# PhucNguyenAH/tacotron2_subword

Measured on AMD Instinct MI355X. Metric: mel_frames_per_sec_train, higher is better.
Workload: dtype bf16; 1 GPU; BERT_Tacotron2 default hparams (SMA), full training iteration fwd+loss+bwd+clip+Adam, B=64/GPU, 100 phones, 60 sub-word tokens, 400 frames, 80-mel; global_batch=64, frames_per_item=400, parallelism=dp1, torch_ops=loss reductions, cat/transpose copies, persistent_chains=True, recurrent_steps_bf16=True

## Files before the change

include/t2amd.h:

```cpp
#ifndef T2AMD_H
#define T2AMD_H
#include <stddef.h>
#include <stdint.h>

#ifdef __cplusplus
extern "C" {
#endif

#define T2_ATTN_SMA 0
#define T2_ATTN_LSA 1
#define T2_ATTN_DCA 4
#define T2_ATTN_GMM 3
#define T2_ATTN_FWD2 2

enum {
    T2_SITE_PRENET1 = 1, T2_SITE_PRENET2 = 2, T2_SITE_PRENET1_SUB = 3, T2_SITE_PRENET2_SUB = 4,
    T2_SITE_ATT_H = 5, T2_SITE_ATT_C = 6, T2_SITE_ATT_H_SUB = 7, T2_SITE_ATT_C_SUB = 8,
    T2_SITE_DEC_H = 9, T2_SITE_DEC_C = 10, T2_SITE_NOISE = 11, T2_SITE_NOISE_SUB = 12,
    T2_SITE_ENC0 = 16,
    T2_SITE_ENCSUB0 = 20,
    T2_SITE_POSTNET0 = 24
};

const char* t2_last_error(void);
#define T2_ABI_VERSION 4
int t2_version(void);
int t2_chain_status(uint32_t* out_host );
int t2_chain_status_clear(void);
int t2_debug_report_abort(uint32_t code, void* stream);
int t2_debug_occupy(int workgroups, int milliseconds, void* stream);
int t2_chain_claimed(void);
int t2_set_precision(int mode);
int t2_get_precision(void);
int t2_gemm_counts(uint64_t* out_host , int reset);
int t2_set_gemm_split_min_mflop(int mflop);
int t2_set_split_steps(int on);
int t2_get_split_steps(void);
int t2_step_counts(uint64_t* out_host , int reset);
int t2_set_overlap(int on);
int t2_set_chain(int on);
int t2_get_chain(void);
int t2_set_chain_bwd(int on);
int t2_set_gemm_staging(int on);
int t2_set_gemm_fold(int on);
int t2_set_bn_fuse(int on);
int t2_get_bn_fuse(void);
int t2_bn_fuse_counts(uint64_t* out_host , int reset);
int t2_side_join(void* stream);
int t2_defer_counts(uint64_t* out_host , int reset);

typedef struct t2_dims {
    int n_mel;
    int prenet_dim;
    int enc_dim;
    int att_rnn_dim;
    int dec_rnn_dim;
    int att_dim;
    int loc_filters;
    int loc_kernel;
    int attention_kind;
    float p_att_dropout, p_dec_dropout, p_prenet_dropout;
    int n_streams;
    float score_mask_value, score_mask_value_sub;
    int score_mask_given;
} t2_dims;

typedef struct t2_attention_weights {
// ... 159 lines not shown
    float* gates[4];
    float* ws; size_t ws_floats;
} t2_lstm_seq_args;
size_t t2_lstm_seq_chain_ws_floats(int nstreams, int B, int H, int backward);
int t2_lstm_seq_forward(const t2_lstm_seq_args* a, void* stream);
typedef struct t2_lstm_seq_bwd_args {
    int nstreams, B, T, H;
    const float* w_hh[4]; int reverse[4];
    const float* h[4]; long ldh; const float* c[4]; const float* gates[4];
    const float* dh[4]; long lddh;
    float* dpre[4];
    float* dw_hh[4];
    float* ws; size_t ws_floats;
} t2_lstm_seq_bwd_args;
int t2_lstm_seq_backward(const t2_lstm_seq_bwd_args* a, void* stream);

typedef struct t2_gemm_args {
    const float* A; const float* B; float* C; int M, N, K;
    long sam, sak, sbn, sbk, ldc; int batch; long bsA, bsB, bsC;
    float alpha, beta; const float* bias; int act; int crow_mod; long crow_mul;
    float* ws; size_t ws_bytes; int splitk;
} t2_gemm_args;
int t2_gemm_ex(const t2_gemm_args* a, void* stream);
int t2_prof_gemm(const t2_gemm_args* a, int reps, float* ms_total, float* ms_kernel, void* stream);
enum { T2_GEMM_F32_64 = 0, T2_GEMM_F32_128, T2_GEMM_BF16CONV, T2_GEMM_SRC128, T2_GEMM_SRC256, T2_GEMM_SRC256KM };
enum { T2_GEMM_OPERAND_FP32 = 0, T2_GEMM_OPERAND_STAGED, T2_GEMM_OPERAND_CALLER };
typedef struct t2_gemm_plan_opts {
    int conv_a, conv_b, conv_T, conv_C, fp32_only;
    int a16, b16; long lda16, ldb16; int a16_kmajor, b16_kmajor, split16;
} t2_gemm_plan_opts;
typedef struct t2_gemm_plan_info {
    int kernel; const char* name;
    int split;
    int splitk, kchunks;
    int a_src, b_src;
    size_t stage_bytes_a, stage_bytes_b;
} t2_gemm_plan_info;
int t2_gemm_plan(const t2_gemm_args* a, const t2_gemm_plan_opts* opts, t2_gemm_plan_info* out);
int t2_conv_handoff_plan(const t2_gemm_args* a, const t2_gemm_plan_opts* opts, int* taken, t2_gemm_plan_info* out);
int t2_colsum(const float* x, long ld, int M, int N, float* out, float* scratch, void* stream);
int t2_mask_btc(float* x, int B, int T, int C, const int32_t* lengths, float fill, void* stream);

typedef struct t2_softdtw_plan_info {
    int threads;
    int rows_per_thread;
    int passes;
// ... 133 lines not shown
```

tacotron2_subword_amd/_lib.py:

```python
from __future__ import annotations

import ctypes as C
import os

import torch

_HERE = os.path.dirname(os.path.abspath(__file__))
LIB_PATH = os.environ.get("T2AMD_LIB") or os.path.join(_HERE, "libt2amd.so")

ATTN_SMA, ATTN_LSA, ATTN_FWD2, ATTN_GMM, ATTN_DCA = 0, 1, 2, 3, 4

SITE = dict(PRENET1=1, PRENET2=2, PRENET1_SUB=3, PRENET2_SUB=4, ATT_H=5, ATT_C=6, ATT_H_SUB=7, ATT_C_SUB=8,
            DEC_H=9, DEC_C=10, NOISE=11, NOISE_SUB=12, ENC0=16, ENCSUB0=20, POSTNET0=24)

_fp = C.POINTER(C.c_float)
_ip = C.POINTER(C.c_int32)


class Dims(C.Structure):
    _fields_ = [("n_mel", C.c_int), ("prenet_dim", C.c_int), ("enc_dim", C.c_int), ("att_rnn_dim", C.c_int),
                ("dec_rnn_dim", C.c_int), ("att_dim", C.c_int), ("loc_filters", C.c_int), ("loc_kernel", C.c_int),
                ("attention_kind", C.c_int), ("p_att_dropout", C.c_float), ("p_dec_dropout", C.c_float),
                ("p_prenet_dropout", C.c_float), ("n_streams", C.c_int),
                ("score_mask_value", C.c_float), ("score_mask_value_sub", C.c_float), ("score_mask_given", C.c_int)]
# ... 99 lines not shown
_I4 = C.c_int * 4


class LstmSeqArgs(C.Structure):
    _fields_ = [("nstreams", C.c_int), ("B", C.c_int), ("T", C.c_int), ("H", C.c_int),
                ("pre", _P4), ("w_hh", _P4), ("reverse", _I4), ("lengths", C.c_void_p),
                ("h", _P4), ("ldh", C.c_long), ("c", _P4), ("gates", _P4), ("ws", C.c_void_p), ("ws_floats", C.c_size_t)]


class LstmSeqBwdArgs(C.Structure):
    _fields_ = [("nstreams", C.c_int), ("B", C.c_int), ("T", C.c_int), ("H", C.c_int),
                ("w_hh", _P4), ("reverse", _I4), ("h", _P4), ("ldh", C.c_long), ("c", _P4), ("gates", _P4),
                ("dh", _P4), ("lddh", C.c_long), ("dpre", _P4), ("dw_hh", _P4), ("ws", C.c_void_p), ("ws_floats", C.c_size_t)]


class GemmArgs(C.Structure):
    _fields_ = [("A", C.c_void_p), ("B", C.c_void_p), ("C", C.c_void_p), ("M", C.c_int), ("N", C.c_int), ("K", C.c_int),
                ("sam", C.c_long), ("sak", C.c_long), ("sbn", C.c_long), ("sbk", C.c_long), ("ldc", C.c_long),
                ("batch", C.c_int), ("bsA", C.c_long), ("bsB", C.c_long), ("bsC", C.c_long),
                ("alpha", C.c_float), ("beta", C.c_float), ("bias", C.c_void_p), ("act", C.c_int),
                ("crow_mod", C.c_int), ("crow_mul", C.c_long), ("ws", C.c_void_p), ("ws_bytes", C.c_size_t), ("splitk", C.c_int)]


class GemmPlanOpts(C.Structure):
    _fields_ = [("conv_a", C.c_int), ("conv_b", C.c_int), ("conv_T", C.c_int), ("conv_C", C.c_int), ("fp32_only", C.c_int),
                ("a16", C.c_int), ("b16", C.c_int), ("lda16", C.c_long), ("ldb16", C.c_long),
                ("a16_kmajor", C.c_int), ("b16_kmajor", C.c_int), ("split16", C.c_int)]


class GemmPlanInfo(C.Structure):
    _fields_ = [("kernel", C.c_int), ("name", C.c_char_p), ("split", C.c_int), ("splitk", C.c_int), ("kchunks", C.c_int),
                ("a_src", C.c_int), ("b_src", C.c_int), ("stage_bytes_a", C.c_size_t), ("stage_bytes_b", C.c_size_t)]


class SoftDtwPlanInfo(C.Structure):
    _fields_ = [("threads", C.c_int), ("rows_per_thread", C.c_int), ("passes", C.c_int),
                ("d_floats", C.c_size_t), ("r_floats", C.c_size_t), ("e_floats", C.c_size_t)]


class SoftDtwDistArgs(C.Structure):
    _fields_ = [("B", C.c_int), ("N", C.c_int), ("M", C.c_int), ("d", C.c_int), ("x", C.c_void_p), ("y", C.c_void_p), ("Ds", C.c_void_p)]


class SoftDtwFwdArgs(C.Structure):
    _fields_ = [("B", C.c_int), ("N", C.c_int), ("M", C.c_int), ("gamma", C.c_float), ("bandwidth", C.c_float),
                ("D", C.c_void_p), ("Ds", C.c_void_p), ("x_lengths", C.c_void_p), ("y_lengths", C.c_void_p),
# ... 43 lines not shown


class StftPlanInfo(C.Structure):
    _fields_ = [("bins", C.c_int), ("overlap", C.c_int), ("frame_tile", C.c_int), ("bin_tile", C.c_int), ("out_len", C.c_long),
                ("fwd_floats", C.c_size_t), ("inv_floats", C.c_size_t), ("wsq_floats", C.c_size_t), ("packed_bytes", C.c_size_t)]


class StftAnalysisArgs(C.Structure):
    _fields_ = [("B", C.c_int), ("N", C.c_int), ("hop", C.c_int), ("n", C.c_long), ("x", C.c_void_p), ("packed", C.c_void_p),
                ("re", C.c_void_p), ("im", C.c_void_p), ("mag", C.c_void_p), ("phase", C.c_void_p)]


class StftSynthesisArgs(C.Structure):
    _fields_ = [("B", C.c_int), ("N", C.c_int), ("hop", C.c_int), ("nf", C.c_int), ("mode", C.c_int), ("windowed", C.c_int),
                ("a", C.c_void_p), ("b", C.c_void_p), ("bias", C.c_void_p), ("strength", C.c_float),
                ("packed", C.c_void_p), ("y", C.c_void_p)]


STFT_FRAME_TILE = 32
STFT_POLAR, STFT_DENOISE = 0, 1

ABI_VERSION = 4

EXPORTS = ["t2_last_error", "t2_version", "t2_chain_status", "t2_chain_status_clear", "t2_debug_report_abort", "t2_debug_occupy", "t2_chain_claimed", "t2_set_precision", "t2_get_precision", "t2_gemm_counts", "t2_set_gemm_split_min_mflop", "t2_set_split_steps", "t2_get_split_steps", "t2_step_counts", "t2_set_overlap", "t2_set_chain", "t2_get_chain", "t2_set_chain_bwd", "t2_set_gemm_staging", "t2_set_gemm_fold", "t2_set_bn_fuse", "t2_get_bn_fuse", "t2_bn_fuse_counts", "t2_side_join", "t2_defer_counts", "t2_decoder_layout_query", "t2_decoder_forward", "t2_decoder_infer",
           "t2_decoder_bwd_layout_query", "t2_decoder_backward", "t2_prof_enable", "t2_prof_collect", "t2_adam_chunks", "t2_adam_step", "t2_adam_norm",
           "t2_conv_bn_forward", "t2_conv_bn_backward", "t2_embedding_forward", "t2_embedding_backward",
           "t2_lstm_seq_forward", "t2_lstm_seq_backward", "t2_lstm_seq_chain_ws_floats", "t2_gemm_ex", "t2_prof_gemm", "t2_gemm_plan", "t2_conv_handoff_plan", "t2_colsum", "t2_mask_btc",
           "t2_finalize_bct", "t2_mask_bt", "t2_gemm", "t2_rng_keep_mask", "t2_rng_normal",
           "t2_softdtw_plan", "t2_softdtw_dist", "t2_softdtw_forward", "t2_softdtw_backward", "t2_softdtw_dist_backward",
           "t2_hifigan_plan", "t2_hifigan_pack", "t2_hifigan_forward", "t2_vocoder_packed_floats", "t2_vocoder_conv1d", "t2_vocoder_conv_transpose1d",
           "t2_stft_plan", "t2_stft_pack", "t2_stft_analysis", "t2_stft_synthesis"]

_lib = None


def lib() -> C.CDLL:
    global _lib
    if _lib is None:
        if not os.path.exists(LIB_PATH):
            raise RuntimeError(f"{LIB_PATH} is missing: the HIP extension must be built (see __graft_entry__.build); "
                               "there is no CPU fallback for the product path")
        L = C.CDLL(LIB_PATH)
        L.t2_last_error.restype = C.c_char_p
        if L.t2_version() != ABI_VERSION:
            raise RuntimeError(f"{LIB_PATH} speaks ABI version {L.t2_version()}, this binding {ABI_VERSION}: rebuild the library "
                               "(the argument structs differ in size between versions)")
        L.t2_chain_status.argtypes = [C.POINTER(C.c_uint32)]
        L.t2_debug_report_abort.argtypes = [C.c_uint32, C.c_void_p]
        L.t2_debug_occupy.argtypes = [C.c_int, C.c_int, C.c_void_p]
        L.t2_gemm.argtypes = [C.c_void_p, C.c_void_p, C.c_void_p, C.c_int, C.c_int, C.c_int, C.c_long, C.c_long, C.c_long,
                              C.c_long, C.c_long, C.c_void_p, C.c_int, C.c_float, C.c_float, C.c_void_p, C.c_size_t,
                              C.c_int, C.c_void_p]
        L.t2_rng_keep_mask.argtypes = [C.c_uint64, C.c_uint32, C.c_uint32, C.c_float, C.c_void_p, C.c_void_p]
        L.t2_rng_normal.argtypes = [C.c_uint64, C.c_uint32, C.c_uint32, C.c_void_p, C.c_void_p]
        L.t2_decoder_layout_query.argtypes = [C.POINTER(Dims), C.c_int, C.c_int, C.c_int, C.c_int, C.POINTER(DecoderLayout)]
        L.t2_decoder_forward.argtypes = [C.POINTER(Dims), C.POINTER(DecoderWeights), C.POINTER(DecoderFwdArgs), C.c_void_p]
        L.t2_decoder_infer.argtypes = [C.POINTER(Dims), C.POINTER(DecoderWeights), C.POINTER(DecoderInferArgs), C.c_void_p]
        L.t2_decoder_bwd_layout_query.argtypes = [C.POINTER(Dims), C.c_int, C.c_int, C.c_int, C.c_int, C.POINTER(DecoderBwdLayout)]
        L.t2_decoder_backward.argtypes = [C.POINTER(Dims), C.POINTER(DecoderWeights), C.POINTER(DecoderGrads),
                                          C.POINTER(DecoderBwdArgs), C.c_void_p]
        L.t2_conv_bn_forward.argtypes = [C.POINTER(ConvBnArgs), C.c_void_p]
        L.t2_conv_bn_backward.argtypes = [C.POINTER(ConvBnBwdArgs), C.c_void_p]
        L.t2_embedding_forward.argtypes = [C.c_void_p, C.c_void_p, C.c_void_p, C.c_int, C.c_int, C.c_void_p]
        L.t2_embedding_backward.argtypes = [C.c_void_p, C.c_void_p, C.c_void_p, C.c_int, C.c_int, C.c_int, C.c_void_p]
        L.t2_lstm_seq_forward.argtypes = [C.POINTER(LstmSeqArgs), C.c_void_p]
        L.t2_lstm_seq_backward.argtypes = [C.POINTER(LstmSeqBwdArgs), C.c_void_p]
        L.t2_lstm_seq_chain_ws_floats.argtypes, L.t2_lstm_seq_chain_ws_floats.restype = [C.c_int, C.c_int, C.c_int, C.c_int], C.c_size_t
        L.t2_gemm_ex.argtypes = [C.POINTER(GemmArgs), C.c_void_p]
        L.t2_prof_gemm.argtypes = [C.POINTER(GemmArgs), C.c_int, C.POINTER(C.c_float), C.POINTER(C.c_float), C.c_void_p]
        L.t2_gemm_plan.argtypes = [C.POINTER(GemmArgs), C.POINTER(GemmPlanOpts), C.POINTER(GemmPlanInfo)]
        L.t2_conv_handoff_plan.argtypes = [C.POINTER(GemmArgs), C.POINTER(GemmPlanOpts), C.POINTER(C.c_int), C.POINTER(GemmPlanInfo)]
        L.t2_colsum.argtypes = [C.c_void_p, C.c_long, C.c_int, C.c_int, C.c_void_p, C.c_void_p, C.c_void_p]
        L.t2_mask_btc.argtypes = [C.c_void_p, C.c_int, C.c_int, C.c_int, C.c_void_p, C.c_float, C.c_void_p]
        L.t2_prof_enable.argtypes = [C.c_int]
        L.t2_gemm_counts.argtypes = [C.POINTER(C.c_uint64), C.c_int]
        L.t2_set_split_steps.argtypes = [C.c_int]
        L.t2_step_counts.argtypes = [C.POINTER(C.c_uint64), C.c_int]
        L.t2_bn_fuse_counts.argtypes = [C.POINTER(C.c_uint64), C.c_int]
        L.t2_defer_counts.argtypes = [C.POINTER(C.c_uint64), C.c_int]
        L.t2_set_gemm_split_min_mflop.argtypes = [C.c_int]
        L.t2_prof_collect.argtypes = [C.c_int, C.POINTER(C.c_double), C.POINTER(C.c_int)]
        L.t2_finalize_bct.argtypes = [C.c_void_p, C.c_void_p, C.c_int, C.c_int, C.c_int, C.c_void_p, C.c_float, C.c_void_p]
        L.t2_mask_bt.argtypes = [C.c_void_p, C.c_int, C.c_int, C.c_void_p, C.c_float, C.c_void_p]
        L.t2_softdtw_plan.argtypes = [C.c_int, C.c_int, C.c_int, C.c_float, C.c_int, C.POINTER(SoftDtwPlanInfo)]
        L.t2_softdtw_dist.argtypes = [C.POINTER(SoftDtwDistArgs), C.c_void_p]
        L.t2_softdtw_forward.argtypes = [C.POINTER(SoftDtwFwdArgs), C.c_void_p]
        L.t2_softdtw_backward.argtypes = [C.POINTER(SoftDtwBwdArgs), C.c_void_p]
        L.t2_softdtw_dist_backward.argtypes = [C.POINTER(SoftDtwDistBwdArgs), C.c_void_p]
        L.t2_hifigan_plan.argtypes = [C.POINTER(HifiganConfig), C.c_int, C.c_int, C.POINTER(HifiganPlanInfo)]
        L.t2_hifigan_pack.argtypes = [C.POINTER(HifiganConfig), C.POINTER(C.c_void_p), C.POINTER(C.c_void_p), C.c_int, C.c_void_p, C.c_void_p]
        L.t2_hifigan_forward.argtypes = [C.POINTER(HifiganConfig), C.POINTER(HifiganFwdArgs), C.c_void_p]
# ... 224 lines not shown
    out = (C.c_uint64 * 6)()
    check(lib().t2_step_counts(out, int(bool(reset))))
    return tuple(int(v) for v in out)


def gemm_plan(args: GemmArgs, **opts) -> dict:
    o, info = GemmPlanOpts(**opts), GemmPlanInfo()
    check(lib().t2_gemm_plan(C.byref(args), C.byref(o), C.byref(info)))
    return dict(kernel=info.kernel, name=info.name.decode(), split=bool(info.split), splitk=info.splitk, kchunks=info.kchunks,
                a_src=info.a_src, b_src=info.b_src, stage_bytes_a=info.stage_bytes_a, stage_bytes_b=info.stage_bytes_b)


def conv_handoff_plan(args: GemmArgs, **opts) -> dict:
    o, info, taken = GemmPlanOpts(**opts), GemmPlanInfo(), C.c_int(0)
    check(lib().t2_conv_handoff_plan(C.byref(args), C.byref(o), C.byref(taken), C.byref(info)))
    return dict(taken=bool(taken.value), kernel=info.kernel, name=info.name.decode(), split=bool(info.split), splitk=info.splitk,
                kchunks=info.kchunks, a_src=info.a_src, b_src=info.b_src, stage_bytes_a=info.stage_bytes_a, stage_bytes_b=info.stage_bytes_b)


def set_gemm_fold(on: bool) -> None:
    check(lib().t2_set_gemm_fold(1 if on else 0))


def set_bn_fuse(on: bool) -> None:
    check(lib().t2_set_bn_fuse(1 if on else 0))


def get_bn_fuse() -> bool:
    return bool(lib().t2_get_bn_fuse())


def bn_fuse_counts(reset: bool = False):
    out = (C.c_uint64 * 3)()
    check(lib().t2_bn_fuse_counts(out, int(bool(reset))))
    return tuple(int(v) for v in out)


def defer_counts(reset: bool = False):
    out = (C.c_uint64 * 2)()
    check(lib().t2_defer_counts(out, int(bool(reset))))
    return tuple(int(v) for v in out)


def set_gemm_split_min_mflop(mflop: int = -1) -> None:
    check(lib().t2_set_gemm_split_min_mflop(int(mflop)))

# ... 44 lines not shown
```

tacotron2_subword_amd/csrc/c_api.hip:

```cpp
#include <fcntl.h>
#include <stdarg.h>
#include <stdio.h>
#include <sys/file.h>
#include <unistd.h>
#include <stdlib.h>
#include <string.h>

#include "../../include/t2amd.h"
#include "kernels.h"
#include "driver.h"

static thread_local char g_err[512] = "";

void t2_set_error(const char* fmt, ...) {
    va_list ap;
    va_start(ap, fmt);
    vsnprintf(g_err, sizeof(g_err), fmt, ap);
    va_end(ap);
}

#include <algorithm>
#include <mutex>
#include <vector>

// ... 165 lines not shown
    set_precision(mode);
    return 0;
}
int t2_get_precision(void) { return get_precision(); }
int t2_set_gemm_split_min_mflop(int mflop) { set_gemm_split_min_mflop(mflop); return 0; }
int t2_gemm_counts(uint64_t* out_host, int reset) {
    T2_REQUIRE(out_host, "null argument");
    gemm_counts(out_host, reset);
    return 0;
}
int t2_set_split_steps(int on) { g_split_steps = on != 0; return 0; }
int t2_get_split_steps(void) { return g_split_steps; }
int t2_step_counts(uint64_t* out_host, int reset) {
    T2_REQUIRE(out_host, "null argument");
    for (int i = 0; i < 6; ++i) { out_host[i] = g_step_counts[i]; if (reset) g_step_counts[i] = 0; }
    return 0;
}
int t2_set_overlap(int on) { g_overlap = on != 0; return 0; }
int t2_set_chain(int on) { g_chain = on != 0; return 0; }
int t2_get_chain(void) { return g_chain; }
int t2_set_chain_bwd(int on) { g_chain_bwd = on != 0; return 0; }
int t2_set_gemm_staging(int on) { set_gemm_staging(on); return 0; }
int t2_set_gemm_fold(int on) { set_gemm_fold(on); return 0; }
int t2_set_bn_fuse(int on) { set_bn_fuse(on); return 0; }
int t2_get_bn_fuse(void) { return get_bn_fuse(); }
int t2_bn_fuse_counts(uint64_t* out_host, int reset) {
    T2_REQUIRE(out_host, "null argument");
    bn_fuse_counts(out_host, reset);
    return 0;
}
int t2_defer_counts(uint64_t* out_host, int reset) {
    T2_REQUIRE(out_host, "null argument");
    for (int i = 0; i < 2; ++i) { out_host[i] = g_defer_counts[i]; if (reset) g_defer_counts[i] = 0; }
    return 0;
}
int t2_side_join(void* stream) {
    Side* side = nullptr;
    T2_TRY(side_get(&side));
    hipEvent_t e;
    T2_TRY(side_event(*side, 0, &e));
    T2_CHECK_HIP(hipEventRecord(e, side->s));
    T2_CHECK_HIP(hipStreamWaitEvent((hipStream_t)stream, e, 0));
    return 0;
}

int t2_conv_bn_forward(const t2_conv_bn_args* a, void* stream) {
// ... 124 lines not shown
        w.A = a->reverse[i] ? a->dpre[i] : a->dpre[i] + rowsB * 4 * H; w.sam = 1; w.sak = 4 * H;
        w.B = a->reverse[i] ? a->h[i] + rowsB * a->ldh : a->h[i]; w.sbk = a->ldh; w.sbn = 1;
        w.C = a->dw_hh[i]; w.ldc = H; w.M = 4 * H; w.N = H; w.K = (T - 1) * B;
        w.ws = gws; w.ws_bytes = gws_bytes;
        T2_TRY(gemm(w, s));
    }
    return 0;
}

static GemmDesc desc_of(const t2_gemm_args& a) {
    GemmDesc g = gemm_desc();
    g.A = a.A; g.B = a.B; g.C = a.C; g.M = a.M; g.N = a.N; g.K = a.K;
    g.sam = a.sam; g.sak = a.sak; g.sbn = a.sbn; g.sbk = a.sbk; g.ldc = a.ldc;
    g.batch = a.batch > 0 ? a.batch : 1; g.bsA = a.bsA; g.bsB = a.bsB; g.bsC = a.bsC;
    g.alpha = a.alpha; g.beta = a.beta; g.bias1 = a.bias; g.act = a.act;
    g.crow_mod = a.crow_mod; g.crow_mul = a.crow_mul;
    g.ws = a.ws; g.ws_bytes = a.ws_bytes; g.splitk = a.splitk;
    return g;
}
int t2_gemm_ex(const t2_gemm_args* a, void* stream) {
    T2_REQUIRE(a, "null argument");
    return gemm(desc_of(*a), (hipStream_t)stream);
}
static GemmDesc desc_of(const t2_gemm_args& a, const t2_gemm_plan_opts* o) {
    GemmDesc g = desc_of(a);
    if (o) {
        g.conv_a = o->conv_a; g.conv_b = o->conv_b; g.conv_T = o->conv_T; g.conv_C = o->conv_C; g.fp32_only = o->fp32_only;
        const __bf16* copy = reinterpret_cast<const __bf16*>(uintptr_t(256));
        if (o->a16) { g.A16 = copy; g.lda16 = o->lda16; g.a16_kmajor = o->a16_kmajor; }
        if (o->b16) { g.B16 = copy; g.ldb16 = o->ldb16; g.b16_kmajor = o->b16_kmajor; }
        g.split16 = o->split16;
    }
    return g;
}
static t2_gemm_plan_info info_of(const GemmPlan& p) {
    return t2_gemm_plan_info{(int)p.kernel, gemm_plan_name(p), p.split, p.splitk, p.kchunks, (int)p.a.src, (int)p.b.src, p.a.bytes, p.b.bytes};
}
int t2_gemm_plan(const t2_gemm_args* a, const t2_gemm_plan_opts* o, t2_gemm_plan_info* out) {
    T2_REQUIRE(a && out, "null argument");
    GemmPlan p;
    T2_TRY(gemm_plan(desc_of(*a, o), &p));
    *out = info_of(p);
    return 0;
}
int t2_conv_handoff_plan(const t2_gemm_args* a, const t2_gemm_plan_opts* o, int* taken, t2_gemm_plan_info* out) {
    T2_REQUIRE(a && taken && out, "null argument");
// ... 208 lines not shown
```

tacotron2_subword_amd/csrc/gemm.hip:

```cpp
#include "kernels.h"
#include <cstdlib>
#include <algorithm>
#include <type_traits>

namespace t2 {

static int g_precision = 0;
static int env_int(const char* name, int dflt) { const char* v = getenv(name); return v && *v ? atoi(v) : dflt; }
static int g_stage = env_int("T2_GEMM_STAGE", 1);
void set_gemm_staging(int on) { g_stage = on != 0; }
static int g_fold = env_int("T2_GEMM_FOLD", 1);
void set_gemm_fold(int on) { g_fold = on != 0; }
int get_gemm_fold() { return g_fold; }
constexpr int kStageMin = 256;
constexpr int kSplitMinMflopDefault = 2147;
static double g_split_min_flop = 1e6 * kSplitMinMflopDefault;
void set_gemm_split_min_mflop(int mflop) { g_split_min_flop = 1e6 * (mflop < 0 ? kSplitMinMflopDefault : mflop); }
void set_precision(int p) { g_precision = p; }
int get_precision() { return g_precision; }
static uint64_t g_counts[4] = {0, 0, 0, 0};
void gemm_counts(uint64_t* out, int reset) {
    for (int i = 0; i < 4; ++i) { out[i] = g_counts[i]; if (reset) g_counts[i] = 0; }
}

namespace {

constexpr int BK = 16;

struct GemmK {
    GemmDesc d;
    int kchunks;
    int avec, bvec;
    int xcd_swizzle;
};

__device__ __forceinline__ float apply_act(float v, int act) {
// ... 214 lines not shown
        int s = 0;
        for (; s + 8 <= d.splitk; s += 8) {
            float v[8];
#pragma unroll
            for (int j = 0; j < 8; ++j) v[j] = d.ws[(long)(s + j) * total + i];
#pragma unroll
            for (int j = 0; j < 8; ++j) acc += v[j];
        }
        if (s + 4 <= d.splitk) {
            float v[4];
#pragma unroll
            for (int j = 0; j < 4; ++j) v[j] = d.ws[(long)(s + j) * total + i];
#pragma unroll
            for (int j = 0; j < 4; ++j) acc += v[j];
            s += 4;
        }
        for (; s < d.splitk; ++s) acc += d.ws[(long)s * total + i];
        const int bz = (int)(i / ((long)d.M * d.N));
        const long rem = i - (long)bz * d.M * d.N;
        const int m = (int)(rem / d.N), n = (int)(rem % d.N);
        epilogue_store<decltype(cmap)::value>(d, d.C + (long)bz * d.bsC, m, n, acc, key);
    }
    });
}


typedef __bf16 bf16x8 __attribute__((ext_vector_type(8)));
constexpr int BK16 = 64, PK16 = BK16;
__device__ __forceinline__ int swz16(int row, int slot) { return row * PK16 + ((slot ^ ((row ^ (row >> 2)) & 7)) << 3); }

__device__ __forceinline__ bf16x8 pack8(const f32x4& lo, const f32x4& hi) {
    bf16x8 v;
#pragma unroll
    for (int j = 0; j < 4; ++j) { v[j] = (__bf16)lo[j]; v[4 + j] = (__bf16)hi[j]; }
    return v;
}

__device__ __forceinline__ void load16_kc(const float* __restrict__ base, long srow, int row0, int nrows, int k0, int kend, int vec,
                                          ConvAddr cv, bf16x8 (&regs)[4]) {
    if (cv.T && row0 + 128 <= nrows && k0 + BK16 <= kend) {
        f32x4 lo[4], hi[4];
        bool ok[4];
#pragma unroll
        for (int i = 0; i < 4; ++i) {
            const int q = threadIdx.x + i * 256, row = row0 + (q >> 3), k = k0 + (q & 7) * 8;
            const int dk = k / cv.C, ci = k - dk * cv.C, t = row % cv.T + dk - cv.pad;
// ... 893 lines not shown

int choose_splitk(const GemmDesc& d, bool tile256, long tiles, int kch, size_t ws_bytes) {
    if (!(d.ws && d.beta == 0.f)) return 1;
    int sp = 1;
    if (tile256) {
        const int nkt = kch / 4;
        if (d.splitk > 0) sp = std::min(d.splitk, std::max(1, nkt / 2));
        else if (tiles < 512) {
            double best = 0.0;
            for (int c = 1; c <= 16; ++c) {
                if (c > 1 && nkt / c < 16) break;
                const long wgs = tiles * c, rounds = (wgs + 255) / 256;
                const double eff = (double)wgs / (256.0 * rounds);
                if (eff > best * 1.05) { best = eff; sp = c; }
            }
        }
    } else if (d.splitk > 0) sp = d.splitk;
    else if (tiles < 512 && kch >= 64) sp = std::min((int)((1024 + tiles - 1) / tiles), kch / 16);
    const size_t per = (size_t)d.batch * d.M * d.N * sizeof(float);
    if ((size_t)sp * per > ws_bytes) sp = (int)(ws_bytes / per);
    return std::max(sp, 1);
}

int run_gemm(const GemmDesc& d, const GemmPlan& p, hipStream_t s) {
    GemmK g{};
    g.d = d;
    g.kchunks = p.kchunks; g.avec = p.avec; g.bvec = p.bvec;
    if (d.conv_a) { g.d.sam = 0; g.d.sak = 1; }
    if (d.conv_b) { g.d.sbk = 0; g.d.sbn = 1; }
    if (d.drop_mstride == 0) g.d.drop_mstride = (uint32_t)d.N;
    g.d.K = p.K; g.d.conv_C = p.conv_C; g.d.splitk = p.splitk;
    const size_t staged = p.a.bytes + p.b.bytes;
    if (staged) { g.d.ws = reinterpret_cast<float*>(reinterpret_cast<unsigned char*>(d.ws) + staged); g.d.ws_bytes = d.ws_bytes - staged; }
    const int tile = p.kernel == GemmKernel::f32_64 ? 64 : p.kernel >= GemmKernel::src256 ? 256 : 128;
    const dim3 grid((d.N + tile - 1) / tile, (d.M + tile - 1) / tile, d.batch * p.splitk);
    if (gemm_reads_bf16_copies(p.kernel)) {
        __bf16* a16 = reinterpret_cast<__bf16*>(d.ws), * b16 = reinterpret_cast<__bf16*>(reinterpret_cast<unsigned char*>(d.ws) + p.a.bytes);
        if (p.a.src == GemmSrc::staged) T2_TRY_RC(stage_planned(d.A, p.a, p.split, a16, s));
        if (p.b.src == GemmSrc::staged) T2_TRY_RC(stage_planned(d.B, p.b, p.split, b16, s));
        const __bf16* pa = p.a.src == GemmSrc::caller ? d.A16 : a16, * pb = p.b.src == GemmSrc::caller ? d.B16 : b16;
        if (p.kernel == GemmKernel::src256km && d.conv_b) T2_TRY_RC((launch_bf16src256<false, true, true>(g, pa, p.a.ld, pb, p.b.ld, grid, s)));
        else if (p.kernel == GemmKernel::src256km) T2_TRY_RC((launch_bf16src256<false, true, false>(g, pa, p.a.ld, pb, p.b.ld, grid, s)));
        else if (p.kernel == GemmKernel::src256 && d.conv_a) T2_TRY_RC((launch_bf16src256<true, false, false>(g, pa, p.a.ld, pb, p.b.ld, grid, s)));
        else if (p.kernel == GemmKernel::src256) T2_TRY_RC((launch_bf16src256<false, false, false>(g, pa, p.a.ld, pb, p.b.ld, grid, s)));
        else if (d.conv_a) T2_TRY_RC((launch_bf16src<true, 2, 2, 2, 2, 2>(g, pa, p.a.ld, pb, p.b.ld, grid, s)));
        else T2_TRY_RC((launch_bf16src<false, 2, 2, 2, 2, 2>(g, pa, p.a.ld, pb, p.b.ld, grid, s)));
    } else {
        using Kernel = void (*)(GemmK);
        static const Kernel bf16conv[] = {gemm_bf16_kernel<true, true>, gemm_bf16_kernel<true, false>, gemm_bf16_kernel<false, true>, gemm_bf16_kernel<false, false>};
        static const Kernel f32_64[] = {gemm_kernel<64, 64, true, true>, gemm_kernel<64, 64, true, false>, gemm_kernel<64, 64, false, true>, gemm_kernel<64, 64, false, false>};
        static const Kernel f32_128[] = {gemm_kernel<128, 128, true, true>, gemm_kernel<128, 128, true, false>, gemm_kernel<128, 128, false, true>, gemm_kernel<128, 128, false, false>};
        const bool conv16 = p.kernel == GemmKernel::bf16conv;
        const size_t smem = conv16 ? (size_t)4 * 128 * PK16 * sizeof(__bf16) : 0;
        const Kernel kernel = (conv16 ? bf16conv : p.kernel == GemmKernel::f32_64 ? f32_64 : f32_128)[(g.d.sak == 1 ? 0 : 2) + (g.d.sbk == 1 ? 0 : 1)];
        hipLaunchKernelGGL(kernel, grid, dim3(256), smem, s, g);
    }
    T2_LAUNCH_CHECK();
    if (p.splitk > 1) {
        const long total = (long)d.batch * d.M * d.N;
        int blocks = (int)((total + 255) / 256);
        if (blocks > 2048) blocks = 2048;
        hipLaunchKernelGGL(splitk_reduce_kernel, dim3(blocks), dim3(256), 0, s, g.d);
        T2_LAUNCH_CHECK();
    }
    return 0;
}

}

int stage_bf16(const float* src, bool kc, long ld, __bf16* dst, int rows, int K, hipStream_t s) {
    T2_REQUIRE(rows > 0 && K > 0 && rows % 64 == 0 && K % 64 == 0 && ld % 4 == 0 && aligned16(src) && aligned16(dst),
               "stage_bf16: rows=%d K=%d ld=%ld must be whole 64-tiles of 16-byte aligned rows", rows, K, ld);
    return stage_operand(src, kc, ld, dst, rows, K, s);
}

int stage_split_bf16(const float* src, bool kc, long ld, __bf16* dst, int rows, int K, int lo_slot, int row_group, hipStream_t s) {
    T2_REQUIRE(rows > 0 && K > 0 && rows % 64 == 0 && K % 64 == 0 && ld % 4 == 0 && aligned16(src) && aligned16(dst) &&
               (lo_slot == 1 || lo_slot == 2) && row_group >= 0 && (!row_group || (kc && rows % row_group == 0)),
               "stage_split_bf16: rows=%d K=%d ld=%ld must be whole 64-tiles of 16-byte aligned rows", rows, K, ld);
    return stage_split_operand(src, kc, ld, dst, rows, K, lo_slot, row_group, s);
}

int stage_planned(const float* src, const GemmOperandPlan& o, bool split, __bf16* dst, hipStream_t s) {
    return split ? stage_split_operand(src, o.kc, o.ld_src, dst, o.rows, o.K, o.lo_slot, o.row_group, s)
                 : stage_operand(src, o.kc, o.ld_src, dst, o.rows, o.K, s);
}

// ... 81 lines not shown
    T2_TRY_RC(check_gemm(d));
    *out = plan_gemm(d);
    T2_REQUIRE((long)d.batch * out->splitk <= 65535, "gemm: batch*splitk too large (%d*%d)", d.batch, out->splitk);
    return 0;
}

bool gemm_handoff(const GemmDesc& plain, const GemmDesc& offered, GemmPlan* plan) {
    const GemmPlan p0 = plan_gemm(plain);
    if (plan) *plan = p0;
    if (g_precision != 1 || !gemm_reads_bf16_copies(p0.kernel) || !(offered.A16 || offered.B16)) return false;
    if ((offered.A16 && p0.a.src != GemmSrc::staged) || (offered.B16 && p0.b.src != GemmSrc::staged)) return false;
    const GemmPlan p1 = plan_gemm(offered);
    if (p1.kernel != p0.kernel || p1.split != p0.split || p1.splitk != p0.splitk || p1.kchunks != p0.kchunks) return false;
    if ((offered.A16 && p1.a.src != GemmSrc::caller) || (offered.B16 && p1.b.src != GemmSrc::caller)) return false;
    if (plan) *plan = p1;
    return true;
}

int gemm(const GemmDesc& d, hipStream_t s) {
    GemmPlan p;
    T2_TRY_RC(gemm_plan(d, &p));
    static const int g_log = env_int("T2_GEMM_LOG", 0);
    if (g_log)
        fprintf(stderr, "t2gemm M=%d N=%d K=%d batch=%d %s%s kernel=%s splitk=%d stageA=%d stageB=%d convA=%d convB=%d beta=%g\n", d.M, d.N, d.K, d.batch,
                d.conv_a || d.sak == 1 ? "A[m][k]" : "A[k][m]", !d.conv_b && d.sbk == 1 ? " B[n][k]" : " B[k][n]", gemm_plan_name(p),
                p.splitk, p.a.src == GemmSrc::staged, p.b.src == GemmSrc::staged, d.conv_a, d.conv_b, (double)d.beta);
    ++g_counts[p.split ? 3 : gemm_reads_bf16_copies(p.kernel) ? 2 : p.kernel == GemmKernel::bf16conv ? 1 : 0];
    return run_gemm(d, p, s);
}

}
```

tacotron2_subword_amd/csrc/kernels.h:

```cpp
#pragma once
#include "common.h"

namespace t2 {

enum Act : int { ACT_NONE = 0, ACT_RELU = 1, ACT_TANH = 2 };

struct GemmDesc {
    const float* A; const float* B; float* C;
    int M, N, K;
    long sam, sak;
    long sbn, sbk;
    long ldc;
    int batch; long bsA, bsB, bsC;
    float alpha, beta;
    const float* bias1; const float* bias2;
    int act;
    float drop_p; uint64_t seed; uint32_t site;
    uint32_t drop_base, drop_mstride;
    float* ws; size_t ws_bytes;
    int splitk;
    int conv_a, conv_b, conv_T, conv_C, conv_pad;
    int fp32_only;
    const __bf16* A16; long lda16;
    const __bf16* B16; long ldb16;
// ... 25 lines not shown
};
struct GemmPlan {
    GemmKernel kernel;
    bool split;
    int splitk, kchunks;
    int K, conv_C;
    GemmOperandPlan a, b;
    int avec, bvec;
};
GemmPlan plan_gemm(const GemmDesc& d);
int gemm_plan(const GemmDesc& d, GemmPlan* out);
bool gemm_handoff(const GemmDesc& plain, const GemmDesc& offered, GemmPlan* plan = nullptr);
const char* gemm_plan_name(const GemmPlan& p);
int stage_planned(const float* src, const GemmOperandPlan& o, bool split, __bf16* dst, hipStream_t s);
int stage_bf16(const float* src, bool kc, long ld, __bf16* dst, int rows, int K, hipStream_t s);
int stage_split_bf16(const float* src, bool kc, long ld, __bf16* dst, int rows, int K, int lo_slot, int row_group, hipStream_t s);
void set_precision(int p);
int get_precision();
void gemm_counts(uint64_t* out, int reset);
void set_gemm_split_min_mflop(int mflop);
void set_gemm_staging(int on);
void set_gemm_fold(int on);
int get_gemm_fold();

constexpr int kMaxSeg = 6;
struct LstmSeg { const float* x; long ldx; const float* w; long ldw; int k; };
struct LstmStream {
    LstmSeg seg[kMaxSeg]; int nseg;
    const float* pre; long ldpre;
    const float* bias1; const float* bias2;
    const float* c_prev; long ldc_prev;
    float* gates; long ldgates;
    float* c_new; long ldc_new;
    float* h_out; long ldh_out;
    float* h_out2; long ldh_out2;
    float* c_out; long ldc_out;
    uint32_t site_h, site_c; uint32_t idx_base, idx_bstride;
    const int* lengths; int t;
    const float* wq; int A; float* qpart;
    const __bf16* x16; long ldx16; const __bf16* w16; long ldw16; int k16;
    __bf16* h16_out; long ldh16;
    __bf16* h16_out2; long ldh16_2;
    const float* xs; long ldxs; const __bf16* w16lo;
};
constexpr int kMaxLstmStreams = 4;
struct LstmStepDesc { LstmStream st[kMaxLstmStreams]; int nstreams; int B, H; float drop_p; uint64_t seed; };
// ... 345 lines not shown
```

Baseline: 1.056 million mel-frames/s.

## Add vectorized wide and column-mapped split-K reduction kernels

Replaces the scalar split-K reduction with a planner that picks a float4-vectorized kernel which sums several partial slabs per thread with unrolled loads. A second variant handles column-remapped outputs by reordering results through shared memory so stores stay coalesced. Both target the memory-bound reduction pass that follows split-K GEMMs. An env/API toggle keeps the old path available, and a standalone reduce entry point is exposed. The new kernels add more template instantiations and alignment conditions that decide which path runs.

New measurement: 1.061 million mel-frames/s, median of 6. No clear change (+0.5%).

```diff
diff --git a/include/t2amd.h b/include/t2amd.h
--- a/include/t2amd.h
+++ b/include/t2amd.h
@@ -43,6 +43,7 @@
 int t2_set_chain_bwd(int on);
 int t2_set_gemm_staging(int on);
 int t2_set_gemm_fold(int on);
+int t2_set_splitk_reduce(int wide);
 int t2_set_bn_fuse(int on);
 int t2_get_bn_fuse(void);
 int t2_bn_fuse_counts(uint64_t* out_host , int reset);
@@ -248,6 +249,13 @@
     float* ws; size_t ws_bytes; int splitk;
 } t2_gemm_args;
 int t2_gemm_ex(const t2_gemm_args* a, void* stream);
+typedef struct t2_splitk_reduce_opts {
+    const float* bias2; const float* r1_m; const float* r1_n;
+    float drop_p; uint64_t seed; uint32_t site, drop_base, drop_mstride;
+    int ccol_mod, ccol_mul;
+} t2_splitk_reduce_opts;
+int t2_splitk_reduce(const t2_gemm_args* a, int splitk, void* stream);
+int t2_splitk_reduce_ex(const t2_gemm_args* a, const t2_splitk_reduce_opts* opts, int splitk, void* stream);
 int t2_prof_gemm(const t2_gemm_args* a, int reps, float* ms_total, float* ms_kernel, void* stream);
 enum { T2_GEMM_F32_64 = 0, T2_GEMM_F32_128, T2_GEMM_BF16CONV, T2_GEMM_SRC128, T2_GEMM_SRC256, T2_GEMM_SRC256KM };
 enum { T2_GEMM_OPERAND_FP32 = 0, T2_GEMM_OPERAND_STAGED, T2_GEMM_OPERAND_CALLER };
diff --git a/tacotron2_subword_amd/_lib.py b/tacotron2_subword_amd/_lib.py
--- a/tacotron2_subword_amd/_lib.py
+++ b/tacotron2_subword_amd/_lib.py
@@ -145,6 +145,12 @@
                 ("crow_mod", C.c_int), ("crow_mul", C.c_long), ("ws", C.c_void_p), ("ws_bytes", C.c_size_t), ("splitk", C.c_int)]
 
 
+class SplitkReduceOpts(C.Structure):
+    _fields_ = [("bias2", C.c_void_p), ("r1_m", C.c_void_p), ("r1_n", C.c_void_p),
+                ("drop_p", C.c_float), ("seed", C.c_uint64), ("site", C.c_uint32), ("drop_base", C.c_uint32), ("drop_mstride", C.c_uint32),
+                ("ccol_mod", C.c_int), ("ccol_mul", C.c_int)]
+
+
 class GemmPlanOpts(C.Structure):
     _fields_ = [("conv_a", C.c_int), ("conv_b", C.c_int), ("conv_T", C.c_int), ("conv_C", C.c_int), ("fp32_only", C.c_int),
                 ("a16", C.c_int), ("b16", C.c_int), ("lda16", C.c_long), ("ldb16", C.c_long),
@@ -234,10 +240,10 @@
 
 ABI_VERSION = 4
 
-EXPORTS = ["t2_last_error", "t2_version", "t2_chain_status", "t2_chain_status_clear", "t2_debug_report_abort", "t2_debug_occupy", "t2_chain_claimed", "t2_set_precision", "t2_get_precision", "t2_gemm_counts", "t2_set_gemm_split_min_mflop", "t2_set_split_steps", "t2_get_split_steps", "t2_step_counts", "t2_set_overlap", "t2_set_chain", "t2_get_chain", "t2_set_chain_bwd", "t2_set_gemm_staging", "t2_set_gemm_fold", "t2_set_bn_fuse", "t2_get_bn_fuse", "t2_bn_fuse_counts", "t2_side_join", "t2_defer_counts", "t2_decoder_layout_query", "t2_decoder_forward", "t2_decoder_infer",
+EXPORTS = ["t2_last_error", "t2_version", "t2_chain_status", "t2_chain_status_clear", "t2_debug_report_abort", "t2_debug_occupy", "t2_chain_claimed", "t2_set_precision", "t2_get_precision", "t2_gemm_counts", "t2_set_gemm_split_min_mflop", "t2_set_split_steps", "t2_get_split_steps", "t2_step_counts", "t2_set_overlap", "t2_set_chain", "t2_get_chain", "t2_set_chain_bwd", "t2_set_gemm_staging", "t2_set_gemm_fold", "t2_set_splitk_reduce", "t2_set_bn_fuse", "t2_get_bn_fuse", "t2_bn_fuse_counts", "t2_side_join", "t2_defer_counts", "t2_decoder_layout_query", "t2_decoder_forward", "t2_decoder_infer",
            "t2_decoder_bwd_layout_query", "t2_decoder_backward", "t2_prof_enable", "t2_prof_collect", "t2_adam_chunks", "t2_adam_step", "t2_adam_norm",
            "t2_conv_bn_forward", "t2_conv_bn_backward", "t2_embedding_forward", "t2_embedding_backward",
-           "t2_lstm_seq_forward", "t2_lstm_seq_backward", "t2_lstm_seq_chain_ws_floats", "t2_gemm_ex", "t2_prof_gemm", "t2_gemm_plan", "t2_conv_handoff_plan", "t2_colsum", "t2_mask_btc",
+           "t2_lstm_seq_forward", "t2_lstm_seq_backward", "t2_lstm_seq_chain_ws_floats", "t2_gemm_ex", "t2_splitk_reduce", "t2_splitk_reduce_ex", "t2_prof_gemm", "t2_gemm_plan", "t2_conv_handoff_plan", "t2_colsum", "t2_mask_btc",
            "t2_finalize_bct", "t2_mask_bt", "t2_gemm", "t2_rng_keep_mask", "t2_rng_normal",
            "t2_softdtw_plan", "t2_softdtw_dist", "t2_softdtw_forward", "t2_softdtw_backward", "t2_softdtw_dist_backward",
            "t2_hifigan_plan", "t2_hifigan_pack", "t2_hifigan_forward", "t2_vocoder_packed_floats", "t2_vocoder_conv1d", "t2_vocoder_conv_transpose1d",
@@ -279,6 +285,8 @@
         L.t2_lstm_seq_backward.argtypes = [C.POINTER(LstmSeqBwdArgs), C.c_void_p]
         L.t2_lstm_seq_chain_ws_floats.argtypes, L.t2_lstm_seq_chain_ws_floats.restype = [C.c_int, C.c_int, C.c_int, C.c_int], C.c_size_t
         L.t2_gemm_ex.argtypes = [C.POINTER(GemmArgs), C.c_void_p]
+        L.t2_splitk_reduce.argtypes = [C.POINTER(GemmArgs), C.c_int, C.c_void_p]
+        L.t2_splitk_reduce_ex.argtypes = [C.POINTER(GemmArgs), C.POINTER(SplitkReduceOpts), C.c_int, C.c_void_p]
         L.t2_prof_gemm.argtypes = [C.POINTER(GemmArgs), C.c_int, C.POINTER(C.c_float), C.POINTER(C.c_float), C.c_void_p]
         L.t2_gemm_plan.argtypes = [C.POINTER(GemmArgs), C.POINTER(GemmPlanOpts), C.POINTER(GemmPlanInfo)]
         L.t2_conv_handoff_plan.argtypes = [C.POINTER(GemmArgs), C.POINTER(GemmPlanOpts), C.POINTER(C.c_int), C.POINTER(GemmPlanInfo)]
@@ -549,6 +557,14 @@
     check(lib().t2_set_gemm_fold(1 if on else 0))
 
 
+def set_splitk_reduce(wide: bool) -> None:
+    check(lib().t2_set_splitk_reduce(1 if wide else 0))
+
+
+def splitk_reduce(args: GemmArgs, splitk: int, **opts) -> None:
+    check(lib().t2_splitk_reduce_ex(C.byref(args), C.byref(SplitkReduceOpts(**opts)), splitk, stream()))
+
+
 def set_bn_fuse(on: bool) -> None:
     check(lib().t2_set_bn_fuse(1 if on else 0))
 
diff --git a/tacotron2_subword_amd/csrc/c_api.hip b/tacotron2_subword_amd/csrc/c_api.hip
--- a/tacotron2_subword_amd/csrc/c_api.hip
+++ b/tacotron2_subword_amd/csrc/c_api.hip
@@ -211,6 +211,7 @@
 int t2_set_chain_bwd(int on) { g_chain_bwd = on != 0; return 0; }
 int t2_set_gemm_staging(int on) { set_gemm_staging(on); return 0; }
 int t2_set_gemm_fold(int on) { set_gemm_fold(on); return 0; }
+int t2_set_splitk_reduce(int wide) { set_splitk_reduce(wide); return 0; }
 int t2_set_bn_fuse(int on) { set_bn_fuse(on); return 0; }
 int t2_get_bn_fuse(void) { return get_bn_fuse(); }
 int t2_bn_fuse_counts(uint64_t* out_host, int reset) {
@@ -381,6 +382,17 @@
     T2_REQUIRE(a, "null argument");
     return gemm(desc_of(*a), (hipStream_t)stream);
 }
+int t2_splitk_reduce_ex(const t2_gemm_args* a, const t2_splitk_reduce_opts* o, int splitk, void* stream) {
+    T2_REQUIRE(a, "null argument");
+    GemmDesc g = desc_of(*a);
+    if (o) {
+        g.bias2 = o->bias2; g.r1_m = o->r1_m; g.r1_n = o->r1_n;
+        g.drop_p = o->drop_p; g.seed = o->seed; g.site = o->site; g.drop_base = o->drop_base; g.drop_mstride = o->drop_mstride;
+        g.ccol_mod = o->ccol_mod; g.ccol_mul = o->ccol_mul;
+    }
+    return splitk_reduce(g, splitk, (hipStream_t)stream);
+}
+int t2_splitk_reduce(const t2_gemm_args* a, int splitk, void* stream) { return t2_splitk_reduce_ex(a, nullptr, splitk, stream); }
 static GemmDesc desc_of(const t2_gemm_args& a, const t2_gemm_plan_opts* o) {
     GemmDesc g = desc_of(a);
     if (o) {
diff --git a/tacotron2_subword_amd/csrc/gemm.hip b/tacotron2_subword_amd/csrc/gemm.hip
--- a/tacotron2_subword_amd/csrc/gemm.hip
+++ b/tacotron2_subword_amd/csrc/gemm.hip
@@ -12,6 +12,8 @@
 static int g_fold = env_int("T2_GEMM_FOLD", 1);
 void set_gemm_fold(int on) { g_fold = on != 0; }
 int get_gemm_fold() { return g_fold; }
+static int g_wide = env_int("T2_SPLITK_WIDE", 1);
+void set_splitk_reduce(int wide) { g_wide = wide != 0; }
 constexpr int kStageMin = 256;
 constexpr int kSplitMinMflopDefault = 2147;
 static double g_split_min_flop = 1e6 * kSplitMinMflopDefault;
@@ -272,6 +274,110 @@
         epilogue_store<decltype(cmap)::value>(d, d.C + (long)bz * d.bsC, m, n, acc, key);
     }
     });
+}
+
+template <int G, int S>
+__device__ __forceinline__ void sum_partials(const f32x4* __restrict__ ws, const unsigned (&g)[G], size_t slab4, int splitk, f32x4 (&acc)[G]) {
+#pragma unroll
+    for (int j = 0; j < G; ++j) acc[j] = f32x4{0.f, 0.f, 0.f, 0.f};
+    for (int s = 0; s < splitk; s += S) {
+        const int r = splitk - s;
+        f32x4 v[G][S];
+        if (r >= S) {
+#pragma unroll
+            for (int t = 0; t < S; ++t)
+#pragma unroll
+                for (int j = 0; j < G; ++j) v[j][t] = ws[(size_t)(s + t) * slab4 + g[j]];
+#pragma unroll
+            for (int j = 0; j < G; ++j)
+#pragma unroll
+                for (int t = 0; t < S; ++t) acc[j] += v[j][t];
+        } else {
+#pragma unroll
+            for (int t = 0; t < S - 1; ++t)
+                if (t < r)
+#pragma unroll
+                    for (int j = 0; j < G; ++j) v[j][t] = ws[(size_t)(s + t) * slab4 + g[j]];
+#pragma unroll
+            for (int j = 0; j < G; ++j)
+#pragma unroll
+                for (int t = 0; t < S - 1; ++t)
+                    if (t < r) acc[j] += v[j][t];
+        }
+    }
+}
+
+template <int G, int S>
+__global__ __launch_bounds__(256) void splitk_reduce_wide_kernel(GemmDesc d) {
+    const RngKey key = rng_key(d.seed, d.site);
+    const unsigned n4 = (unsigned)d.N >> 2, groups = (unsigned)d.M * n4, bz = blockIdx.y;
+    const size_t slab4 = (size_t)groups * d.batch;
+    const f32x4* __restrict__ ws = reinterpret_cast<const f32x4*>(d.ws) + (size_t)bz * groups;
+    float* C = d.C + (long)bz * d.bsC;
+    const bool vec = (reinterpret_cast<uintptr_t>(C) & 15) == 0 && d.ldc % 4 == 0 && !d.ccol_mod && d.beta == 0.f;
+    for (unsigned g0 = blockIdx.x * (G * 256u) + threadIdx.x; g0 < groups; g0 += gridDim.x * (G * 256u)) {
+        unsigned g[G];
+#pragma unroll
+        for (int j = 0; j < G; ++j) g[j] = min(g0 + j * 256u, groups - 1);
+        f32x4 acc[G];
+        sum_partials<G, S>(ws, g, slab4, d.splitk, acc);
+#pragma unroll
+        for (int j = 0; j < G; ++j) {
+            if (g0 + j * 256u >= groups) break;
+            const int m = (int)(g[j] / n4), n = (int)(g[j] - (unsigned)m * n4) * 4;
+            f32x4 v = acc[j];
+            if (vec) {
+#pragma unroll
+                for (int c = 0; c < 4; ++c) v[c] = epilogue_value(d, m, n + c, v[c], key);
+                const long mo = d.crow_mod ? (long)(m % d.crow_mod) * d.crow_mul + m / d.crow_mod : (long)m;
+                *reinterpret_cast<f32x4*>(C + mo * d.ldc + n) = v;
+            } else {
+                with_col_map(d, [&](auto cmap) {
+#pragma unroll
+                    for (int c = 0; c < 4; ++c) epilogue_store<decltype(cmap)::value>(d, C, m, n + c, v[c], key);
+                });
+            }
+        }
+    }
+}
+
+constexpr int kMapLds = 4096;
+template <int G, int S>
+__global__ __launch_bounds__(256) void splitk_reduce_mapped_kernel(GemmDesc d, int cc, int nchunks, unsigned tasks) {
+    __shared__ __attribute__((aligned(16))) float run[kMapLds];
+    const RngKey key = rng_key(d.seed, d.site);
+    const unsigned mod = d.ccol_mod, mul = d.ccol_mul, n4 = (unsigned)d.N >> 2;
+    const size_t slab4 = (size_t)d.batch * d.M * n4;
+    const f32x4* __restrict__ ws = reinterpret_cast<const f32x4*>(d.ws);
+    for (unsigned task = blockIdx.x; task < tasks; task += gridDim.x) {
+        const unsigned row = task / nchunks, c0 = (task - row * nchunks) * cc;
+        const int bz = (int)(row / (unsigned)d.M), m = (int)(row - (unsigned)bz * d.M);
+        const unsigned cw = min((unsigned)cc, mod - c0), q4 = cw >> 2, ngroups = q4 * mul;
+        const unsigned base4 = row * n4 + (c0 >> 2);
+        for (unsigned g0 = threadIdx.x; g0 < ngroups; g0 += G * blockDim.x) {
+            unsigned g[G], tap[G], q[G];
+#pragma unroll
+            for (int j = 0; j < G; ++j) {
+                const unsigned gi = min(g0 + j * blockDim.x, ngroups - 1);
+                tap[j] = gi / q4; q[j] = gi - tap[j] * q4;
+                g[j] = base4 + tap[j] * (mod >> 2) + q[j];
+            }
+            f32x4 acc[G];
+            sum_partials<G, S>(ws, g, slab4, d.splitk, acc);
+#pragma unroll
+            for (int j = 0; j < G; ++j) {
+                if (g0 + j * blockDim.x >= ngroups) break;
+                const int n = (int)(tap[j] * mod + c0 + 4 * q[j]);
+#pragma unroll
+                for (int c = 0; c < 4; ++c) run[(4 * q[j] + c) * mul + tap[j]] = epilogue_value(d, m, n + c, acc[j][c], key);
+            }
+        }
+        __syncthreads();
+        const long mo = d.crow_mod ? (long)(m % d.crow_mod) * d.crow_mul + m / d.crow_mod : (long)m;
+        f32x4* pc = reinterpret_cast<f32x4*>(d.C + (long)bz * d.bsC + mo * d.ldc + (long)c0 * mul);
+        for (unsigned i = threadIdx.x; i < ngroups; i += blockDim.x) pc[i] = reinterpret_cast<const f32x4*>(run)[i];
+        __syncthreads();
+    }
 }
 
 
@@ -1211,6 +1317,69 @@
     return std::max(sp, 1);
 }
 
+struct ReducePlan {
+    int kind;
+    int G, S;
+    dim3 grid; int threads;
+    int cc, nchunks; unsigned tasks;
+};
+constexpr int kReduceBlocks = 2048;
+constexpr int kReduceWaves = 2048;
+ReducePlan plan_splitk_reduce(const GemmDesc& d) {
+    ReducePlan r{};
+    const long total = (long)d.batch * d.M * d.N;
+    r.grid = dim3((unsigned)std::min<long>((total + 255) / 256, kReduceBlocks));
+    r.threads = 256;
+    if (!g_wide || d.N % 4 != 0 || !aligned16(d.ws) || total >= (1l << 31)) return r;
+    const long groups = total / 4, waves = (groups + 63) / 64;
+    if (d.splitk >= 32 && waves < kReduceWaves) return r;
+    r.S = d.splitk <= 4 ? 4 : d.splitk <= 8 ? 8 : 16;
+    r.G = d.splitk <= 4 ? 4 : d.splitk <= 8 ? 2 : 1;
+    while (r.G > 1 && waves / r.G < kReduceWaves) r.G >>= 1;
+    const bool mapped = d.ccol_mod && d.ccol_mod % 4 == 0 && d.ccol_mul == d.N / d.ccol_mod && d.ccol_mul <= kMapLds / 4 &&
+                        d.beta == 0.f && aligned16(d.C) && d.ldc % 4 == 0 && d.bsC % 4 == 0;
+    if (!mapped) {
+        const long tiles = ((long)d.M * (d.N / 4) + r.G * 256 - 1) / (r.G * 256), passes = (tiles + kReduceBlocks - 1) / kReduceBlocks;
+        r.kind = 1;
+        r.grid = dim3((unsigned)((tiles + passes - 1) / passes), d.batch);
+        return r;
+    }
+    const int mod = d.ccol_mod, mul = d.ccol_mul;
+    const long rows = (long)d.batch * d.M;
+    int cc = std::min(mod, (kMapLds / mul) & ~3);
+    auto chunks = [&](int c) { return (mod + c - 1) / c; };
+    while (rows * chunks(cc) < 1024) {
+        const int half = ((cc + 1) / 2 + 3) & ~3;
+        if (half >= cc || half / 4 * mul < 128) break;
+        cc = half;
+    }
+    r.kind = 2; r.cc = cc; r.nchunks = chunks(cc); r.tasks = (unsigned)(rows * r.nchunks);
+    r.threads = std::min(256, (((cc / 4 * mul + r.G - 1) / r.G + 63) / 64) * 64);
+    const long passes = ((long)r.tasks + kReduceBlocks - 1) / kReduceBlocks;
+    r.grid = dim3((unsigned)((r.tasks + passes - 1) / passes));
+    return r;
+}
+
+template <int G, int S>
+void launch_reduce(const GemmDesc& d, const ReducePlan& r, hipStream_t s) {
+    if (r.kind == 1) hipLaunchKernelGGL((splitk_reduce_wide_kernel<G, S>), r.grid, dim3(256), 0, s, d);
+    else hipLaunchKernelGGL((splitk_reduce_mapped_kernel<G, S>), r.grid, dim3(r.threads), 0, s, d, r.cc, r.nchunks, r.tasks);
+}
+int launch_splitk_reduce(const GemmDesc& d, hipStream_t s) {
+    const ReducePlan r = plan_splitk_reduce(d);
+    switch (r.kind ? r.G * 100 + r.S : 0) {
+        case 0: hipLaunchKernelGGL(splitk_reduce_kernel, r.grid, dim3(256), 0, s, d); break;
+        case 404: launch_reduce<4, 4>(d, r, s); break;
+        case 204: launch_reduce<2, 4>(d, r, s); break;
+        case 104: launch_reduce<1, 4>(d, r, s); break;
+        case 208: launch_reduce<2, 8>(d, r, s); break;
+        case 108: launch_reduce<1, 8>(d, r, s); break;
+        default: launch_reduce<1, 16>(d, r, s); break;
+    }
+    T2_LAUNCH_CHECK();
+    return 0;
+}
+
 int run_gemm(const GemmDesc& d, const GemmPlan& p, hipStream_t s) {
     GemmK g{};
     g.d = d;
@@ -1245,13 +1414,7 @@
         hipLaunchKernelGGL(kernel, grid, dim3(256), smem, s, g);
     }
     T2_LAUNCH_CHECK();
-    if (p.splitk > 1) {
-        const long total = (long)d.batch * d.M * d.N;
-        int blocks = (int)((total + 255) / 256);
-        if (blocks > 2048) blocks = 2048;
-        hipLaunchKernelGGL(splitk_reduce_kernel, dim3(blocks), dim3(256), 0, s, g.d);
-        T2_LAUNCH_CHECK();
-    }
+    if (p.splitk > 1) T2_TRY_RC(launch_splitk_reduce(g.d, s));
     return 0;
 }
 
@@ -1379,11 +1542,23 @@
     T2_TRY_RC(gemm_plan(d, &p));
     static const int g_log = env_int("T2_GEMM_LOG", 0);
     if (g_log)
-        fprintf(stderr, "t2gemm M=%d N=%d K=%d batch=%d %s%s kernel=%s splitk=%d stageA=%d stageB=%d convA=%d convB=%d beta=%g\n", d.M, d.N, d.K, d.batch,
+        fprintf(stderr, "t2gemm M=%d N=%d K=%d batch=%d %s%s kernel=%s splitk=%d stageA=%d stageB=%d convA=%d convB=%d beta=%g colmap=%d:%d\n", d.M, d.N, d.K, d.batch,
                 d.conv_a || d.sak == 1 ? "A[m][k]" : "A[k][m]", !d.conv_b && d.sbk == 1 ? " B[n][k]" : " B[k][n]", gemm_plan_name(p),
-                p.splitk, p.a.src == GemmSrc::staged, p.b.src == GemmSrc::staged, d.conv_a, d.conv_b, (double)d.beta);
+                p.splitk, p.a.src == GemmSrc::staged, p.b.src == GemmSrc::staged, d.conv_a, d.conv_b, (double)d.beta, d.ccol_mod, d.ccol_mul);
     ++g_counts[p.split ? 3 : gemm_reads_bf16_copies(p.kernel) ? 2 : p.kernel == GemmKernel::bf16conv ? 1 : 0];
     return run_gemm(d, p, s);
 }
 
-}
+int splitk_reduce(const GemmDesc& d, int splitk, hipStream_t s) {
+    GemmDesc g = d;
+    g.A = g.B = nullptr; g.K = 1; g.sam = g.sak = g.sbn = g.sbk = 1; g.conv_a = g.conv_b = 0;
+    T2_TRY_RC(check_gemm(g));
+    const size_t total = (size_t)d.batch * d.M * d.N;
+    T2_REQUIRE(splitk >= 1 && (long)d.batch * splitk <= 65535 && d.ws && d.ws_bytes / sizeof(float) / splitk >= total,
+               "splitk_reduce: %d slabs of %zu floats need scratch (%zu bytes given)", splitk, total, d.ws_bytes);
+    g.splitk = splitk;
+    if (g.drop_mstride == 0) g.drop_mstride = (uint32_t)d.N;
+    return launch_splitk_reduce(g, s);
+}
+
+}
diff --git a/tacotron2_subword_amd/csrc/kernels.h b/tacotron2_subword_amd/csrc/kernels.h
--- a/tacotron2_subword_amd/csrc/kernels.h
+++ b/tacotron2_subword_amd/csrc/kernels.h
@@ -71,6 +71,8 @@
 void set_gemm_staging(int on);
 void set_gemm_fold(int on);
 int get_gemm_fold();
+void set_splitk_reduce(int wide);
+int splitk_reduce(const GemmDesc& d, int splitk, hipStream_t s);
 
 constexpr int kMaxSeg = 6;
 struct LstmSeg { const float* x; long ldx; const float* w; long ldw; int k; };
```
